# H2muller/CROPSR

Measured on AMD Instinct MI355X. Metric: gRNAs scored/sec, higher is better.
Workload: dtype f64

## Files before the change

cropsr_amd/csrc/crp_kernels.hip:

```cpp
#include <hip/hip_runtime.h>
#include <stdint.h>

#include <type_traits>

#include "crp_kernels.h"
#include "crp_score.h"
#include "crp_score_generic.h"

namespace crp {

static constexpr uint64_t ALL = ~0ull;

__device__ __forceinline__ uint32_t funnel(uint32_t hi, uint32_t lo, int s)
{
    return __builtin_amdgcn_alignbit(hi, lo, (uint32_t)s);
}
__device__ __forceinline__ uint64_t pair64(uint32_t hi, uint32_t lo) { return ((uint64_t)hi << 32) | lo; }

__device__ __forceinline__ uint64_t ahead(uint64_t cur, uint64_t next, int d)
{
    const uint32_t c0 = (uint32_t)cur, c1 = (uint32_t)(cur >> 32), n0 = (uint32_t)next, n1 = (uint32_t)(next >> 32);
    if (d < 32) return pair64(funnel(n0, c1, d), funnel(c1, c0, d));
    return pair64(funnel(n1, n0, d - 32), funnel(n0, c1, d - 32));
}
__device__ __forceinline__ uint64_t behind(uint64_t prev, uint64_t cur, int e)
{
    const uint32_t p0 = (uint32_t)prev, p1 = (uint32_t)(prev >> 32), c0 = (uint32_t)cur, c1 = (uint32_t)(cur >> 32);
    if (e == 32) return pair64(c0, p1);
    if (e < 32) return pair64(funnel(c1, c0, 32 - e), funnel(c0, p1, 32 - e));
    return pair64(funnel(c0, p1, 64 - e), funnel(p1, p0, 64 - e));
}

constexpr int DPP_WAVE_SHL1 = 0x130, DPP_WAVE_SHR1 = 0x138;
template <int CTRL>
__device__ __forceinline__ uint64_t wave_shift(uint64_t x, uint64_t edge)
{
    const uint32_t lo = (uint32_t)__builtin_amdgcn_update_dpp((int)(uint32_t)edge, (int)(uint32_t)x, CTRL, 0xf, 0xf, false);
    const uint32_t hi =
        (uint32_t)__builtin_amdgcn_update_dpp((int)(uint32_t)(edge >> 32), (int)(uint32_t)(x >> 32), CTRL, 0xf, 0xf, false);
    return pair64(hi, lo);
}

__device__ __forceinline__ uint64_t wave_inclusive_scan(uint64_t v)
{
    const int lane = threadIdx.x & 63;
#pragma unroll
    for (int d = 1; d < 64; d <<= 1) {
        const uint64_t o = __shfl_up(v, d, 64);
        if (lane >= d) v += o;
    }
    return v;
}

template <int CTRL, int ROW_MASK>
__device__ __forceinline__ uint32_t dpp_add(uint32_t v)
{
    return v + (uint32_t)__builtin_amdgcn_update_dpp(0, (int)v, CTRL, ROW_MASK, 0xf, true);
}

__device__ __forceinline__ uint32_t wave_inclusive_scan_u32(uint32_t v)
{
    v = dpp_add<0x111, 0xf>(v);
    v = dpp_add<0x112, 0xf>(v);
    v = dpp_add<0x114, 0xf>(v);
    v = dpp_add<0x118, 0xf>(v);
    v = dpp_add<0x142, 0xa>(v);
    v = dpp_add<0x143, 0xc>(v);
    return v;
}

__device__ __forceinline__ uint32_t wave_sum_u32(uint32_t v)
{
    return (uint32_t)__builtin_amdgcn_readlane((int)wave_inclusive_scan_u32(v), 63);
}

struct TileScan {
    uint32_t ex_plus, ex_minus, n_plus, n_minus;
};

template <int WAVES>
__device__ __forceinline__ TileScan block_exclusive_scan(uint32_t v16, uint32_t *wave_tot)
{
    const int lane = threadIdx.x & 63, wave = __builtin_amdgcn_readfirstlane((int)(threadIdx.x >> 6));
    const uint32_t inc16 = wave_inclusive_scan_u32(v16);
    if (lane == 63) wave_tot[wave] = inc16;
    __syncthreads();
    uint32_t base_p = 0, base_m = 0, tot_p = 0, tot_m = 0;
#pragma unroll
    for (int w = 0; w < WAVES; ++w) {
        const uint32_t t = (uint32_t)__builtin_amdgcn_readfirstlane((int)wave_tot[w]);
        if (w < wave) {
            base_p += t & 0xffffu;
            base_m += t >> 16;
        }
        tot_p += t & 0xffffu;
        tot_m += t >> 16;
    }
    const uint32_t ex16 = inc16 - v16;
    return TileScan{base_p + (ex16 & 0xffffu), base_m + (ex16 >> 16), tot_p, tot_m};
}

__device__ __forceinline__ void derive(uint64_t hi, uint64_t lo, uint64_t up, uint64_t ac, uint64_t &g,
                                       uint64_t &c, uint64_t &v)
{
    g = hi & lo & up & ac;
    c = hi & ~lo & up & ac;
    v = hi & lo & ~up & ~ac;
}

__device__ __forceinline__ void masks_of(uint64_t g_c, uint64_t g_n, uint64_t c_c, uint64_t c_n, uint64_t v_p,
                                         uint64_t v_c, uint64_t v_n, int l, uint64_t &mplus, uint64_t &mminus)
{
    mplus = ahead(g_c, g_n, 1) & ahead(g_c, g_n, 2) & ~behind(v_p, v_c, l + 5);
    uint64_t m = c_c & ahead(c_c, c_n, 1) & ~ahead(v_c, v_n, 2) & ~behind(v_p, v_c, 2);
    if (l > 8) m &= ~ahead(v_c, v_n, l - 8);
    mminus = m;
}

template <int WPT>
__device__ __forceinline__ void own_words_and_masks(const Planes &pl, uint64_t n_words_padded, uint64_t w0, int lane, int l,
                                                    uint64_t (&q)[4][WPT], uint64_t (&mp)[WPT], uint64_t (&mm)[WPT])
{
    static_assert(WPT == 1 || WPT == 2, "one or two words per owning lane");
    const uint64_t wa = w0 + (uint64_t)WPT * lane;
    if constexpr (WPT == 2) {
#pragma unroll
        for (int p = 0; p < 4; ++p) {
            const ulonglong2 v = *reinterpret_cast<const ulonglong2 *>(pl.plane[p] + wa);
            q[p][0] = v.x;
            q[p][WPT - 1] = v.y;
        }
    } else {
#pragma unroll
        for (int p = 0; p < 4; ++p) q[p][0] = pl.plane[p][wa];
    }
    uint64_t e[4] = {ALL, ALL, 0, 0};
    if (lane == 0 && w0 > 0) {
#pragma unroll
        for (int p = 0; p < 4; ++p) e[p] = pl.plane[p][w0 - 1];
    } else if (lane == 63 && w0 + 64 * WPT < n_words_padded) {
#pragma unroll
        for (int p = 0; p < 4; ++p) e[p] = pl.plane[p][w0 + 64 * WPT];
    }
    uint64_t ga, ca, va, gb, cb, vb, ge, ce, ve;
    derive(q[0][0], q[1][0], q[2][0], q[3][0], ga, ca, va);
    derive(q[0][WPT - 1], q[1][WPT - 1], q[2][WPT - 1], q[3][WPT - 1], gb, cb, vb);
    derive(e[0], e[1], e[2], e[3], ge, ce, ve);
    const uint64_t v_left = wave_shift<DPP_WAVE_SHR1>(vb, ve);
    const uint64_t g_right = wave_shift<DPP_WAVE_SHL1>(ga, ge), c_right = wave_shift<DPP_WAVE_SHL1>(ca, ce),
                   v_right = wave_shift<DPP_WAVE_SHL1>(va, ve);
    if constexpr (WPT == 2) {
        masks_of(ga, gb, ca, cb, v_left, va, vb, l, mp[0], mm[0]);
        masks_of(gb, g_right, cb, c_right, va, vb, v_right, l, mp[WPT - 1], mm[WPT - 1]);
    } else {
        masks_of(ga, g_right, ca, c_right, v_left, va, v_right, l, mp[0], mm[0]);
    }
}

template <class G, int LFIX>
__global__ __launch_bounds__(G::BLOCK) void count_kernel(Planes pl, uint64_t n_words_padded, int l_arg,
                                                         uint2 *__restrict__ tile_cnt)
{
    const int l = LFIX > 0 ? LFIX : l_arg;
    const uint32_t tile = blockIdx.x;
    __shared__ uint64_t wave_tot[G::BLOCK / 64];
    const int lane = threadIdx.x & 63, wave = threadIdx.x >> 6;
    uint64_t c = 0;
    const uint64_t w0 = (uint64_t)tile * G::WORDS + (uint64_t)wave * 64 * G::WPT;
    if (wave < G::OWNERS / 64 && w0 < n_words_padded) {
        uint64_t q[4][G::WPT], mp[G::WPT], mm[G::WPT];
        own_words_and_masks<G::WPT>(pl, n_words_padded, w0, lane, l, q, mp, mm);
#pragma unroll
        for (int k = 0; k < G::WPT; ++k) c += (uint64_t)__popcll(mp[k]) | ((uint64_t)__popcll(mm[k]) << 32);
    }
#pragma unroll
    for (int d = 32; d > 0; d >>= 1) c += __shfl_down(c, d, 64);
    if (lane == 0) wave_tot[wave] = c;
    __syncthreads();
    if (threadIdx.x == 0 && (uint64_t)tile * G::WORDS < n_words_padded) {
        uint64_t t = 0;
#pragma unroll
        for (int w = 0; w < G::BLOCK / 64; ++w) t += wave_tot[w];
        tile_cnt[tile] = make_uint2((uint32_t)t, (uint32_t)(t >> 32));
    }
}

__global__ __launch_bounds__(1024) void tile_scan_kernel(const uint2 *__restrict__ tile_cnt, uint32_t n_tiles,
                                                          uint2 *__restrict__ tile_off,
                                                          uint64_t *__restrict__ totals)
{
    const uint32_t chunk = blockIdx.x;
    constexpr int PER = 8, CHUNK = 1024 * PER;
    __shared__ uint64_t buf[CHUNK];
    __shared__ uint64_t wave_tot[16];
    const int lane = threadIdx.x & 63, wave = threadIdx.x >> 6;
    const uint32_t base = chunk * CHUNK;
    uint64_t carry = 0;
    {
        uint64_t acc = 0;
        const ulonglong2 *cnt2 = reinterpret_cast<const ulonglong2 *>(tile_cnt);
        for (uint32_t i = threadIdx.x; i < base / 2; i += 4096) {
            ulonglong2 c[4];
#pragma unroll
            for (int k = 0; k < 4; ++k) c[k] = cnt2[i + k * 1024];
#pragma unroll
            for (int k = 0; k < 4; ++k) {
                acc += c[k].x + c[k].y;
            }
        }
#pragma unroll
        for (int d = 32; d > 0; d >>= 1) acc += __shfl_xor(acc, d, 64);
        if (lane == 0) wave_tot[wave] = acc;
        __syncthreads();
#pragma unroll
        for (int w = 0; w < 16; ++w) carry += wave_tot[w];
        __syncthreads();
    }
    {
#pragma unroll
        for (int k = 0; k < PER; ++k) {
            const uint32_t i = base + k * 1024 + threadIdx.x;
            uint64_t v = 0;
            if (i < n_tiles) {
                const uint2 c = tile_cnt[i];
                v = (uint64_t)c.x | ((uint64_t)c.y << 32);
            }
            buf[k * 1024 + threadIdx.x] = v;
        }
        __syncthreads();
        uint64_t loc[PER], sum = 0;
#pragma unroll
        for (int k = 0; k < PER; ++k) {
            loc[k] = buf[threadIdx.x * PER + k];
            sum += loc[k];
        }
        const uint64_t inc = wave_inclusive_scan(sum);
        if (lane == 63) wave_tot[wave] = inc;
        __syncthreads();
        uint64_t pre = carry, tot = 0;
#pragma unroll
        for (int w = 0; w < 16; ++w) {
            const uint64_t t = wave_tot[w];
            if (w < wave) pre += t;
            tot += t;
        }
        uint64_t ex = pre + inc - sum;
#pragma unroll
        for (int k = 0; k < PER; ++k) {
            buf[threadIdx.x * PER + k] = ex;
            ex += loc[k];
        }
        carry += tot;
        __syncthreads();
#pragma unroll
        for (int k = 0; k < PER; ++k) {
            const uint32_t i = base + k * 1024 + threadIdx.x;
            const uint64_t v = buf[k * 1024 + threadIdx.x];
            if (i < n_tiles) tile_off[i] = make_uint2((uint32_t)v, (uint32_t)(v >> 32));
        }
    }
    if (threadIdx.x == 0 && base + CHUNK >= n_tiles) {
        totals[0] = carry & 0xffffffffull;
        totals[1] = carry >> 32;
    }
}

__device__ __forceinline__ uint32_t window31(const uint64_t *plane, uint32_t q)
{
    const uint32_t *p32 = reinterpret_cast<const uint32_t *>(plane);
    const uint32_t i = q >> 5;
    return __builtin_amdgcn_alignbit(p32[i + 1], p32[i], q & 31) & 0x7fffffffu;
}

__device__ __forceinline__ uint32_t window32(const uint64_t *plane, uint32_t q)
{
    const uint32_t *p32 = reinterpret_cast<const uint32_t *>(plane);
    const uint32_t i = q >> 5;
    return __builtin_amdgcn_alignbit(p32[i + 1], p32[i], q & 31);
}

__device__ __forceinline__ uint32_t reverse30(uint32_t x) { return __brev(x) >> 2; }

static constexpr uint64_t DESC_AGG = 1ull << 62, DESC_PREFIX = 2ull << 62, DESC_VALUE = (1ull << 62) - 1;

__device__ __forceinline__ uint64_t desc_pack(uint64_t packed32)
{
    return (packed32 & 0x7fffffffull) | ((packed32 >> 32) << 31);
}
__device__ __forceinline__ uint64_t desc_unpack(uint64_t v)
{
    return (v & 0x7fffffffull) | (((v >> 31) & 0x7fffffffull) << 32);
}

constexpr int CHAIN_HEADER_WORDS = 4;
constexpr int LB_DEPTH = 2;

__device__ __forceinline__ void lookback_publish(uint64_t *desc, uint32_t tile, uint64_t total)
{
    const uint64_t tag = tile == 0 ? DESC_PREFIX : DESC_AGG;
    __hip_atomic_store(&desc[tile], tag | desc_pack(total), __ATOMIC_RELAXED, __HIP_MEMORY_SCOPE_AGENT);
}

__device__ __forceinline__ void lookback_load(const uint64_t *desc, int64_t base, uint64_t (&v)[LB_DEPTH])
{
    const int lane = threadIdx.x & 63;
#pragma unroll
    for (int j = 0; j < LB_DEPTH; ++j) {
        const int64_t idx = base - lane - 64 * j;
        v[j] = DESC_PREFIX;
        if (idx >= 0) v[j] = __hip_atomic_load(&desc[idx], __ATOMIC_RELAXED, __HIP_MEMORY_SCOPE_AGENT);
    }
}

__device__ __forceinline__ uint64_t lookback_resolve(uint64_t *desc, uint32_t tile, uint64_t total, uint32_t *fail,
                                                     bool muted, uint32_t timeout_ticks)
{
    const int lane = threadIdx.x & 63;
    if (tile == 0) return 0;
    uint64_t v[LB_DEPTH];
    uint64_t excl = 0;
    int64_t base = (int64_t)tile - 1;
    lookback_load(desc, base, v);
    uint32_t spins = 0;
    uint64_t t_first_stall = 0;
    bool stalled_before = false;
    while (true) {
        uint64_t contrib = 0;
        bool found = false, stall = false;
        int64_t missing = 0;
#pragma unroll
        for (int j = 0; j < LB_DEPTH; ++j) {
            const uint64_t st = v[j] >> 62;
            const uint64_t not_ready = __ballot(st == 0);
            const uint64_t is_prefix = __ballot(st == 2);
            const int p = is_prefix ? __builtin_ctzll(is_prefix) : 64;
            const uint64_t need = p >= 64 ? ~0ull : ((1ull << p) - 1);
            if (!found && !stall) {
                if (not_ready & need) {
                    stall = true;
                    missing = base - 64 * j - __builtin_ctzll(not_ready & need);
                } else {
                    if (lane <= p) contrib += desc_unpack(v[j] & DESC_VALUE);
                    found = p < 64;
                }
            }
        }
        if (stall) {
            while ((__hip_atomic_load(&desc[missing], __ATOMIC_RELAXED, __HIP_MEMORY_SCOPE_AGENT) >> 62) == 0) {
                bool give_up = false;
                if ((spins++ & 15u) == 0) {
                    const uint64_t now = __builtin_amdgcn_s_memrealtime();
                    if (!stalled_before) {
                        t_first_stall = now;
                        stalled_before = true;
                    }
                    give_up = now - t_first_stall > timeout_ticks;
                    give_up |= __hip_atomic_load(fail, __ATOMIC_RELAXED, __HIP_MEMORY_SCOPE_AGENT) != 0;
                }
                if (give_up) {
                    if (lane == 0) {
                        atomicExch(fail, 1u);
                        uint64_t *const host = reinterpret_cast<uint64_t *>(reinterpret_cast<uint64_t *>(fail - 1)[3]);
                        if (host) host[0] = 1ull << 32;
                    }
                    return 0;
                }
                __builtin_amdgcn_s_sleep(8);
            }
        } else {
            excl += pair64(wave_sum_u32((uint32_t)(contrib >> 32)), wave_sum_u32((uint32_t)contrib));
            if (found) break;
            base -= 64 * LB_DEPTH;
        }
        lookback_load(desc, base, v);
    }
    if (lane == 0 && !muted)
        __hip_atomic_store(&desc[tile], DESC_PREFIX | desc_pack(excl + total), __ATOMIC_RELAXED, __HIP_MEMORY_SCOPE_AGENT);
    return excl;
}

struct ChainArgs {
    uint64_t *desc;
    uint32_t *fail;
    uint64_t *totals;
    uint64_t *s_excl;
    uint32_t *s_flag;
    uint32_t tile, n_tiles;
    uint64_t total;
    bool muted;
    uint32_t timeout_ticks;
};

__device__ __forceinline__ void chain_resolve(const ChainArgs &ch)
{
    const uint64_t e = lookback_resolve(ch.desc, ch.tile, ch.total, ch.fail, ch.muted, ch.timeout_ticks);
    if ((threadIdx.x & 63) == 0) {
        *ch.s_excl = e;
        if (ch.tile == ch.n_tiles - 1) {
            const uint64_t all = e + ch.total;
            ch.totals[0] = all & 0xffffffffull;
            ch.totals[1] = all >> 32;
            uint64_t *const host = reinterpret_cast<uint64_t *>(ch.totals[2]);
            if (host) {
                host[1] = all & 0xffffffffull;
                host[2] = all >> 32;
            }
        }
    }
    __hip_atomic_store(ch.s_flag, 1u, __ATOMIC_RELEASE, __HIP_MEMORY_SCOPE_WORKGROUP);
}

struct alignas(16) TabsImage {
    uint64_t exp_tab[256];
    double score_tab[CRP_SCORE_TAB_N];
};
static_assert(sizeof(TabsImage) % 16 == 0, "staged in 16-byte units");
__device__ const TabsImage CRP_TABS = {{
#include "exp_table.inc"
                                       },
                                       CRP_SCORE_TAB_DATA};

__device__ __forceinline__ __amdgpu_buffer_rsrc_t rows_rsrc(void *table, uint64_t cap, uint64_t first, uint32_t skip,
                                                            uint32_t elem)
{
    const uint64_t room = cap > first ? cap - first : 0;
    uint64_t bytes = room ? (room + skip) * elem : 0;
    if (bytes > 0xffffffffull) bytes = 0xffffffffull;
    char *base = reinterpret_cast<char *>(table) + ((int64_t)first - (int64_t)skip) * (int64_t)elem;
    return __builtin_amdgcn_make_buffer_rsrc(base, 0, (int)(uint32_t)bytes, 0x00020000);
}

struct TileStores {
    __amdgpu_buffer_rsrc_t pos[2], score[2], pre[2], seed[2];
};

constexpr int STORE_AUX = 2;
typedef uint32_t u32x2 __attribute__((__vector_size__(2 * sizeof(uint32_t))));
__device__ __forceinline__ u32x2 f64_words(double v)
{
    u32x2 w;
    w[0] = (uint32_t)__double2loint(v);
    w[1] = (uint32_t)__double2hiint(v);
    return w;
}

__device__ __forceinline__ uint64_t uniform64(uint64_t v)
{
    return ((uint64_t)(uint32_t)__builtin_amdgcn_readfirstlane((int)(v >> 32)) << 32) |
           (uint32_t)__builtin_amdgcn_readfirstlane((int)(uint32_t)v);
}

template <bool PRE, bool SEEDS>
__device__ __forceinline__ void tile_stores(TileStores &ts, const HitTables &out, uint64_t off_plus, uint64_t off_minus,
                                            uint32_t n_plus)
{
    ts.pos[0] = rows_rsrc(out.pos_plus, out.cap_plus, off_plus, 0, 4);
    ts.pos[1] = rows_rsrc(out.pos_minus, out.cap_minus, off_minus, n_plus, 4);
    ts.score[0] = rows_rsrc(out.score_plus, out.cap_plus, off_plus, 0, 8);
    ts.score[1] = rows_rsrc(out.score_minus, out.cap_minus, off_minus, n_plus, 8);
    if (PRE) {
        ts.pre[0] = rows_rsrc(out.pre_plus, out.cap_plus, off_plus, 0, 8);
        ts.pre[1] = rows_rsrc(out.pre_minus, out.cap_minus, off_minus, n_plus, 8);
    }
    if (SEEDS) {
        ts.seed[0] = rows_rsrc(out.seed_plus, out.cap_plus, off_plus, 0, 4);
        ts.seed[1] = rows_rsrc(out.seed_minus, out.cap_minus, off_minus, n_plus, 4);
    }
}

__device__ __forceinline__ void peel32(uint32_t m, uint32_t base, uint32_t &addr)
{
    uint32_t b, t;
    uint64_t saved;
    asm volatile(
        "s_mov_b64 %[saved], exec\n\t"
        "v_cmpx_ne_u32_e32 vcc, 0, %[m]\n\t"
        "s_cbranch_execz 2f\n"
        "1:\n\t"
        "v_ffbl_b32_e32 %[b], %[m]\n\t"
        "v_add_u32_e32 %[t], -1, %[m]\n\t"
        "v_or_b32_e32 %[b], %[b], %[base]\n\t"
        "v_and_b32_e32 %[m], %[t], %[m]\n\t"
        "ds_write_b16 %[addr], %[b]\n\t"
        "v_add_u32_e32 %[addr], 2, %[addr]\n\t"
        "v_cmpx_ne_u32_e32 vcc, 0, %[m]\n\t"
        "s_cbranch_execnz 1b\n"
        "2:\n\t"
        "s_mov_b64 exec, %[saved]"
        : [m] "+v"(m), [addr] "+v"(addr), [b] "=&v"(b), [t] "=&v"(t), [saved] "=&s"(saved)
        : [base] "v"(base)
        : "vcc", "memory");
}

template <class G, bool PAM, bool CHAINED, bool PRE, bool SEEDS>
__device__ __forceinline__ void emit_rounds(uint64_t (*sh)[G::WORDS + 2], uint16_t *list, uint64_t *exp_tab, double *score_tab,
                                            const uint64_t (&mp)[G::WPT], const uint64_t (&mm)[G::WPT], uint32_t ex_plus,
                                            uint32_t ex_minus,
                                            uint32_t n_plus, uint32_t n_minus, int l, uint32_t tile_pos,
                                            uint64_t off_plus, uint64_t off_minus, const HitTables &out,
                                            const ChainArgs &ch);

template <class G, bool CHAINED, int LFIX, bool PRE, bool SEEDS>
__global__ __launch_bounds__(G::BLOCK) __attribute__((amdgpu_waves_per_eu(6, 8))) void emit_kernel(
    Planes pl, uint64_t n_words_padded, int l_arg, const uint2 *__restrict__ tile_off, uint64_t *chain,
    uint64_t *__restrict__ chain_next, HitTables out, uint32_t mute_tile, uint32_t timeout_ticks)
{
    const int l = LFIX > 0 ? LFIX : l_arg;
    constexpr int TW = G::WORDS;
    __shared__ uint64_t sh[4][TW + 2];
    __shared__ __attribute__((aligned(16))) uint64_t tabs[256 + CRP_SCORE_TAB_N];
    uint64_t *const exp_tab = tabs;
    double *const score_tab = reinterpret_cast<double *>(tabs + 256);
    __shared__ uint32_t wave_tot[G::BLOCK / 64];
    __shared__ uint64_t s_excl;
    __shared__ uint32_t s_flag;
    __shared__ uint16_t list[G::LIST];
    static_assert(sizeof(sh) + sizeof(tabs) + sizeof(wave_tot) + sizeof(s_excl) + 8 + sizeof(list) <= G::LDS_LIMIT,
                  "workgroups per CU: see the geometry's LIST");

    const int tid = threadIdx.x;
    const uint32_t tile = blockIdx.x;
    if (CHAINED && tid == 0) s_flag = 0;
    const uint64_t t0 = (uint64_t)tile * TW;
    if (CHAINED) __builtin_amdgcn_s_setprio(3);
    uint64_t mp[G::WPT], mm[G::WPT];
#pragma unroll
    for (int k = 0; k < G::WPT; ++k) mp[k] = mm[k] = 0;
    if (G::OWNERS == G::BLOCK || tid < G::OWNERS) {
        const int lane = tid & 63;
        const uint64_t w0 = t0 + (uint64_t)(64 * G::WPT) * (uint64_t)(tid >> 6);
        uint64_t q[4][G::WPT];
        own_words_and_masks<G::WPT>(pl, n_words_padded, w0, lane, l, q, mp, mm);
#pragma unroll
        for (int p = 0; p < 4; ++p)
#pragma unroll
            for (int k = 0; k < G::WPT; ++k) sh[p][1 + G::WPT * tid + k] = q[p][k];
        if (tid < 8) {
            const int p = tid >> 1;
            const uint64_t voidw = (p < 2) ? ALL : 0ull;
            if (tid & 1) sh[p][TW + 1] = t0 + TW < n_words_padded ? pl.plane[p][t0 + TW] : voidw;
            else sh[p][0] = t0 > 0 ? pl.plane[p][t0 - 1] : voidw;
        }
    }
    uint32_t c16 = 0;
#pragma unroll
    for (int k = 0; k < G::WPT; ++k) c16 += (uint32_t)__popcll(mp[k]) | ((uint32_t)__popcll(mm[k]) << 16);
    const TileScan sc = block_exclusive_scan<G::BLOCK / 64>(c16, wave_tot);
    const uint32_t n_plus = sc.n_plus, n_minus = sc.n_minus;
    const uint32_t n_all = n_plus + n_minus;
    const uint64_t total = pair64(n_minus, n_plus);
    uint64_t off_plus = 0, off_minus = 0;
    ChainArgs ch{};
    if (CHAINED) {
        ch = ChainArgs{chain + CHAIN_HEADER_WORDS, reinterpret_cast<uint32_t *>(chain) + 1, chain + 1, &s_excl, &s_flag,
                       tile, gridDim.x, total, tile == mute_tile, timeout_ticks};
        if (tid == 0) {
            if (tile != mute_tile) lookback_publish(ch.desc, tile, total);
            chain_next[CHAIN_HEADER_WORDS + tile] = 0;
            if (tile == 0) chain_next[0] = chain_next[1] = chain_next[2] = 0;
        }
        __builtin_amdgcn_s_setprio(0);
        if (n_all == 0) {
            if (tile == ch.n_tiles - 1 && tid < 64) chain_resolve(ch);
            return;
        }
    } else {
        const uint2 off = tile_off[tile];
        off_plus = off.x;
        off_minus = off.y;
        if (n_all == 0) return;
    }
    constexpr uint32_t TAB_UNITS = (LFIX == 20 ? sizeof(TabsImage) : sizeof(CRP_TABS.exp_tab)) / 16;
    for (uint32_t k = tid; k < TAB_UNITS; k += G::BLOCK)
        reinterpret_cast<uint4 *>(tabs)[k] = reinterpret_cast<const uint4 *>(&CRP_TABS)[k];
    emit_rounds<G, LFIX == 20, CHAINED, PRE, SEEDS>(sh, list, exp_tab, score_tab, mp, mm, sc.ex_plus, sc.ex_minus, n_plus, n_minus, l,
                                                 (uint32_t)(t0 * 64),
                                                 off_plus, off_minus, out, ch);
}

template <class G, bool PAM, bool CHAINED, bool PRE, bool SEEDS>
__device__ __forceinline__ void emit_rounds(uint64_t (*sh)[G::WORDS + 2], uint16_t *list, uint64_t *exp_tab, double *score_tab,
                                            const uint64_t (&mp)[G::WPT], const uint64_t (&mm)[G::WPT], uint32_t ex_plus,
                                            uint32_t ex_minus,
                                            uint32_t n_plus, uint32_t n_minus, int l, uint32_t tile_pos,
                                            uint64_t off_plus, uint64_t off_minus, const HitTables &out,
                                            const ChainArgs &ch)
{
    constexpr uint32_t CAP = G::LIST;
    const int tid = threadIdx.x;
    const uint32_t n_all = n_plus + n_minus;
    TileStores ts;
    bool resolved = !CHAINED;
    if (!CHAINED) tile_stores<PRE, SEEDS>(ts, out, uniform64(off_plus), uniform64(off_minus), n_plus);
    const bool by_strand = n_all > CAP && n_plus <= CAP && n_minus <= CAP;
    const uint32_t list_lds = (uint32_t)(uintptr_t)list;
    uint32_t hi_rank = 0;
    for (uint32_t lo_rank = 0; lo_rank < n_all; lo_rank = hi_rank) {
        hi_rank = by_strand ? (lo_rank == 0 ? n_plus : n_all) : min(lo_rank + CAP, n_all);
        if (lo_rank) __syncthreads();
        const uint32_t rp0 = ex_plus - lo_rank;
        const uint32_t rm0 = ex_minus + (n_plus - lo_rank);
        if (n_all <= CAP || by_strand) {
            const bool with_plus = !by_strand || lo_rank == 0, with_minus = !by_strand || lo_rank != 0;
            uint32_t ap = list_lds + 2 * rp0, am = list_lds + 2 * rm0;
            if (G::OWNERS == G::BLOCK || tid < G::OWNERS) {
#pragma unroll
                for (int k = 0; k < G::WPT; ++k) {
                    const uint32_t wbase = (uint32_t)(tid * G::WPT + k) * 64u;
                    if (with_plus) {
                        peel32((uint32_t)mp[k], wbase, ap);
                        peel32((uint32_t)(mp[k] >> 32), wbase + 32, ap);
                    }
                    if (with_minus) {
                        peel32((uint32_t)mm[k], wbase, am);
                        peel32((uint32_t)(mm[k] >> 32), wbase + 32, am);
                    }
                }
            }
        } else {
            uint32_t rp = rp0, rm = rm0;
#pragma unroll
            for (int k = 0; k < G::WPT; ++k) {
                const uint32_t wbase = (uint32_t)(tid * G::WPT + k) * 64u;
                for (uint64_t m = mp[k]; m; m &= m - 1, ++rp)
                    if (rp < CAP) list[rp] = (uint16_t)(wbase + __builtin_ctzll(m));
                for (uint64_t m = mm[k]; m; m &= m - 1, ++rm)
                    if (rm < CAP) list[rm] = (uint16_t)(wbase + __builtin_ctzll(m));
            }
        }
        __syncthreads();
        const uint32_t n_round = hi_rank - lo_rank;
        struct Hit {
            uint32_t e, r, seed;
            double pre, score;
        };
        struct Fetched {
            uint32_t e, r, h, w, u, a;
        };
        auto fetch = [&](uint32_t k) -> Fetched {
            Fetched f{list[k], lo_rank + k, 0, 0, 0, 0};
            const uint32_t q = 64u + f.e - (f.r >= n_plus ? 2u : PAM ? 27u : (uint32_t)(l + 5));
            if (PAM) {
                f.h = window32(sh[0], q);
                f.w = window32(sh[1], q);
                f.u = window32(sh[2], q);
                f.a = window32(sh[3], q);
            } else if (l >= 20) {
                f.h = window31(sh[0], q);
                f.w = window31(sh[1], q);
                f.u = window31(sh[2], q);
                f.a = window31(sh[3], q);
            }
            return f;
        };
        auto score = [&](const Fetched &f) -> Hit {
            Hit hit{f.e, f.r, SEED_RAW_NONE, -1.0, -1.0};
            const bool minus = hit.r >= n_plus;
            if (PAM) {
                const uint32_t u = f.u;
                uint32_t h = f.h, w = f.w, valid = f.a | u;
                if (!minus) {
                    h = __brev(h);
                    w = __brev(w ^ u);
                    valid = __brev(valid);
                }
                const bool complete = (h & w & ~valid & 0x3fffffffu) == 0;
                if (SEEDS) {
                    if (((valid >> 5) & 0xfffu) == 0xfffu) hit.seed = (((h >> 5) & 0xfffu) << 12) | ((w >> 5) & 0xfffu);
                }
                if (complete) {
                    const uint32_t mG = h & w, mC = h & ~w;
                    const uint32_t mT = ~h & w, mA = ~h & ~w & valid;
                    crp_score_masks<PAM>(mA, mT, mC, mG, exp_tab, score_tab, hit.pre, hit.score);
                }
            } else if (l >= 20) {
                uint32_t h = f.h, w = f.w, u = f.u, a = f.a;
                const uint32_t vd = h & w & ~u & ~a;
                const bool complete = (vd & 0x3fffffffu) == 0 && (l == 20 || (vd >> 30));
                h &= 0x3fffffffu;
                w &= 0x3fffffffu;
                u &= 0x3fffffffu;
                a &= 0x3fffffffu;
                uint32_t valid = a | u;
                if (!minus) {
                    h = reverse30(h);
                    w = reverse30(w ^ u);
                    valid = reverse30(valid);
                }
                static_assert(!SEEDS || PAM, "seed words are emitted by the l = 20 variant only");
                if (complete) {
                    const uint32_t mG = h & w & valid, mC = h & ~w & valid;
                    const uint32_t mT = ~h & w & valid, mA = ~h & ~w & valid;
                    crp_score_masks<PAM>(mA, mT, mC, mG, exp_tab, score_tab, hit.pre, hit.score);
                }
            }
            return hit;
        };
        auto store = [&](const Hit &hit) {
            const uint32_t pos = tile_pos + hit.e;
            const int o4 = (int)(hit.r * 4u), o8 = (int)(hit.r * 8u);
            const bool minus = hit.r >= n_plus;
#pragma unroll
            for (int st = 0; st < 2; ++st) {
                if (minus == (st == 1)) {
                    __builtin_amdgcn_raw_buffer_store_b32(pos, ts.pos[st], o4, 0, STORE_AUX);
                    __builtin_amdgcn_raw_buffer_store_b64(f64_words(hit.score), ts.score[st], o8, 0, STORE_AUX);
                    if (PRE) __builtin_amdgcn_raw_buffer_store_b64(f64_words(hit.pre), ts.pre[st], o8, 0, STORE_AUX);
                    if (SEEDS) __builtin_amdgcn_raw_buffer_store_b32(hit.seed, ts.seed[st], o4, 0, STORE_AUX);
                    if (st == 0) asm volatile("; '+' rows stored" ::: "memory");
                    else asm volatile("; '-' rows stored" ::: "memory");
                }
            }
        };
        auto run_rows = [&](uint32_t k, auto before_first_store) {
            const bool any = k < n_round;
            Hit first{};
            if (any) first = score(fetch(k));
            before_first_store(any);
            if (any) {
                store(first);
                for (k += G::BLOCK; k < n_round; k += G::BLOCK) store(score(fetch(k)));
            }
        };
        if (!CHAINED) {
            run_rows(tid, [](bool) {});
        } else {
            const uint32_t k0 = (uint32_t)(tid & 63) | ((((uint32_t)tid >> 6) + (G::BLOCK / 64 - 1)) % (G::BLOCK / 64)) << 6;
            if (lo_rank == 0 && tid < 64) chain_resolve(ch);
            run_rows(k0, [&](bool any) {
                if (!resolved && __ballot(any)) {
                    while (__builtin_amdgcn_readfirstlane((int)__hip_atomic_load(ch.s_flag, __ATOMIC_ACQUIRE, __HIP_MEMORY_SCOPE_WORKGROUP)) == 0)
                        __builtin_amdgcn_s_sleep(1);
                    const uint64_t e = uniform64(*ch.s_excl);
                    tile_stores<PRE, SEEDS>(ts, out, e & 0xffffffffull, e >> 32, n_plus);
                    resolved = true;
                }
            });
        }
    }
}

__global__ __launch_bounds__(BLOCK) void score30_kernel(const uint8_t *__restrict__ rows, uint64_t n,
                                                         double *__restrict__ pre_out,
                                                         double *__restrict__ score_out)
{
    __shared__ uint64_t exp_tab[256];
    exp_tab[threadIdx.x] = CRP_EXP_TAB[threadIdx.x];
    __syncthreads();
    for (uint64_t i = (uint64_t)blockIdx.x * BLOCK + threadIdx.x; i < n; i += (uint64_t)gridDim.x * BLOCK) {
        const uint8_t *r = rows + 30 * i;
        uint32_t mA = 0, mT = 0, mC = 0, mG = 0;
#pragma unroll
        for (int p = 0; p < 30; ++p) {
            const uint32_t ch = r[p];
            mA |= (uint32_t)(ch == 'A') << p;
            mT |= (uint32_t)(ch == 'T') << p;
            mC |= (uint32_t)(ch == 'C') << p;
            mG |= (uint32_t)(ch == 'G') << p;
        }
        double pre, score;
        crp_score_masks<false>(mA, mT, mC, mG, exp_tab, nullptr, pre, score);
        if (pre_out) pre_out[i] = pre;
        score_out[i] = score;
    }
}

__global__ __launch_bounds__(64) void score30_order_kernel(const uint8_t *__restrict__ rows, uint64_t n, int order,
                                                            double *__restrict__ pre_out,
                                                            double *__restrict__ score_out)
{
    __shared__ uint64_t exp_tab[256];
    for (int k = threadIdx.x; k < 256; k += 64) exp_tab[k] = CRP_EXP_TAB[k];
    __syncthreads();
    for (uint64_t i = (uint64_t)blockIdx.x * 64 + threadIdx.x; i < n; i += (uint64_t)gridDim.x * 64) {
        int8_t code[30];
        for (int p = 0; p < 30; ++p) {
            const uint32_t ch = rows[30 * i + p];
            code[p] = ch == 'A' ? 0 : ch == 'T' ? 1 : ch == 'C' ? 2 : ch == 'G' ? 3 : -1;
        }
        double s1, s2;
        if (order == CRP_ORDER_TAIL2) {
            s1 = crp_sum_tail2<false>(code);
            s2 = crp_sum_tail2<true>(code);
        } else {
            s1 = crp_sum_dot1<false>(code);
            s2 = crp_sum_dot1<true>(code);
        }
        const double pre = (((s1 + s2) + CRP_INTERSECT) + CRP_LOW_GC) * -1.0;
        if (pre_out) pre_out[i] = pre;
        score_out[i] = 1.0 / (1.0 + crp_exp(pre, exp_tab));
    }
}

__host__ __device__ inline uint8_t classify_char(uint32_t ch)
{
    switch (ch) {
        case 'A': case 'U': return 0xC;
        case 'T': return 0xE;
        case 'C': return 0xD;
        case 'G': return 0xF;
        case 'a': return 0x8;
        case 't': return 0xA;
        case 'c': return 0x9;
        case 'g': return 0xB;
        case 'Z': return 0x5;
        default:  return 0x0;
    }
}

__global__ __launch_bounds__(BLOCK) void pack_kernel(const uint8_t *__restrict__ text, uint64_t len,
                                                      uint64_t n_words, uint64_t *__restrict__ hi,
                                                      uint64_t *__restrict__ lo, uint64_t *__restrict__ up,
                                                      uint64_t *__restrict__ ac)
{
    __shared__ uint8_t lut[256];
    __shared__ __attribute__((aligned(16))) uint8_t buf[BLOCK / 64][4096];
    const int tid = threadIdx.x, lane = tid & 63, wave = tid >> 6;
    lut[tid] = classify_char(tid);
    const uint64_t n_groups = (n_words + 63) / 64;
    const uint64_t n_block_iters = (n_groups + BLOCK / 64 - 1) / (BLOCK / 64);
    for (uint64_t bi = blockIdx.x; bi < n_block_iters; bi += gridDim.x) {
        const uint64_t group = bi * (BLOCK / 64) + wave;
        const uint64_t base = group * 4096;
        __syncthreads();
        if (group < n_groups) {
#pragma unroll
            for (int it = 0; it < 4; ++it) {
                const uint64_t off = base + (uint64_t)it * 1024 + (uint64_t)lane * 16;
                uint4 v = make_uint4(0, 0, 0, 0);
                if (off + 16 <= len) {
                    v = *reinterpret_cast<const uint4 *>(text + off);
                } else if (off < len) {
                    uint8_t tmp[16];
                    for (int b = 0; b < 16; ++b) tmp[b] = off + b < len ? text[off + b] : 0;
                    v = *reinterpret_cast<const uint4 *>(tmp);
                }
                *reinterpret_cast<uint4 *>(&buf[wave][it * 1024 + lane * 16]) = v;
            }
        }
        __syncthreads();
        if (group < n_groups) {
            uint64_t w_hi = 0, w_lo = 0, w_up = 0, w_ac = 0;
            for (int t = 0; t < 64; ++t) {
                const uint64_t idx = base + (uint64_t)t * 64 + lane;
                const uint32_t nib = idx < len ? lut[buf[wave][t * 64 + lane]] : 0x3u;
                const uint64_t b0 = __ballot(nib & 1), b1 = __ballot(nib & 2);
                const uint64_t b2 = __ballot(nib & 4), b3 = __ballot(nib & 8);
                if (lane == t) { w_hi = b0; w_lo = b1; w_up = b2; w_ac = b3; }
            }
            const uint64_t w = group * 64 + lane;
            if (w < n_words) { hi[w] = w_hi; lo[w] = w_lo; up[w] = w_up; ac[w] = w_ac; }
        }
    }
}

__global__ __launch_bounds__(BLOCK) void pack_groups_kernel(const uint8_t *__restrict__ text, const PackGroup *__restrict__ groups,
                                                             uint32_t n_groups, uint64_t *__restrict__ hi, uint64_t *__restrict__ lo,
                                                             uint64_t *__restrict__ up, uint64_t *__restrict__ ac)
{
    __shared__ uint8_t lut[256];
    __shared__ __attribute__((aligned(16))) uint8_t buf[BLOCK / 64][4096];
    const int tid = threadIdx.x, lane = tid & 63, wave = tid >> 6;
    lut[tid] = classify_char(tid);
    const uint32_t n_iters = (n_groups + BLOCK / 64 - 1) / (BLOCK / 64);
    for (uint32_t it = blockIdx.x; it < n_iters; it += gridDim.x) {
        const uint32_t g = it * (BLOCK / 64) + wave;
        __syncthreads();
        PackGroup pg{0, 0, 0, 0, 0};
        if (g < n_groups) {
            pg = groups[g];
#pragma unroll
            for (int k = 0; k < 4; ++k)
                *reinterpret_cast<uint4 *>(&buf[wave][k * 1024 + lane * 16]) =
                    *reinterpret_cast<const uint4 *>(text + pg.src + (uint32_t)k * 1024 + (uint32_t)lane * 16);
        }
        __syncthreads();
        if (g < n_groups) {
            uint64_t w_hi = 0, w_lo = 0, w_up = 0, w_ac = 0;
            for (uint32_t t = 0; t < pg.n_words; ++t) {
                const uint32_t idx = t * 64 + lane;
                const uint32_t nib = idx < pg.n_chars ? lut[buf[wave][idx]] : 0x3u;
                const uint64_t b0 = __ballot(nib & 1), b1 = __ballot(nib & 2);
                const uint64_t b2 = __ballot(nib & 4), b3 = __ballot(nib & 8);
                if ((uint32_t)lane == t) { w_hi = b0; w_lo = b1; w_up = b2; w_ac = b3; }
            }
            if ((uint32_t)lane < pg.n_words) {
                const uint64_t w = pg.dst_word + lane;
                hi[w] = w_hi;
                lo[w] = w_lo;
                up[w] = w_up;
                ac[w] = w_ac;
            }
        }
    }
}

template <class G>
static hipError_t launch_count_geo(hipStream_t s, const Planes &pl, uint64_t n_words_padded, int l, uint2 *tile_cnt, uint32_t n_tiles)
{
    if (l == 20)
        hipLaunchKernelGGL((count_kernel<G, 20>), dim3(n_tiles), dim3(G::BLOCK), 0, s, pl, n_words_padded, l, tile_cnt);
    else
        hipLaunchKernelGGL((count_kernel<G, 0>), dim3(n_tiles), dim3(G::BLOCK), 0, s, pl, n_words_padded, l, tile_cnt);
    return hipGetLastError();
}

#define CRP_BY_GEOMETRY(geo, CALL)                 \
    switch (geo) {                                 \
        case GEO_LARGE: return CALL(GeoLarge);     \
        case GEO_SMALL: return CALL(GeoSmall);     \
        default: return hipErrorInvalidValue;      \
    }

hipError_t launch_count(hipStream_t s, int geo, const Planes &pl, uint64_t n_words_padded, int l, uint2 *tile_cnt,
                        uint32_t n_tiles)
{
    if (n_tiles == 0) return hipSuccess;
#define CRP_CALL(G) launch_count_geo<G>(s, pl, n_words_padded, l, tile_cnt, n_tiles)
    CRP_BY_GEOMETRY(geo, CRP_CALL)
#undef CRP_CALL
}

hipError_t launch_tile_scan(hipStream_t s, const uint2 *tile_cnt, uint32_t n_tiles, uint2 *tile_off, uint64_t *totals)
{
    if (n_tiles == 0) return hipSuccess;
    const uint32_t n_chunks = (n_tiles + SCAN_CHUNK_TILES - 1) / SCAN_CHUNK_TILES;
    hipLaunchKernelGGL(tile_scan_kernel, dim3(n_chunks), dim3(1024), 0, s, tile_cnt, n_tiles, tile_off, totals);
    return hipGetLastError();
}

template <class G, bool CHAINED>
static hipError_t launch_emit_variant(hipStream_t s, const Planes &pl, uint64_t n_words_padded, int l, const uint2 *tile_off,
                                      uint64_t *chain, uint64_t *chain_next, const HitTables &out, uint32_t mute_tile,
                                      uint32_t timeout_ticks)
{
    const uint32_t n_tiles = (uint32_t)(n_words_padded / G::WORDS);
    if (n_tiles == 0) return hipSuccess;
    const bool pre = out.pre_plus != nullptr, seeds = out.seed_plus != nullptr;
    if (seeds && l != 20) return hipErrorInvalidValue;
#define CRP_LAUNCH(LFIX, PRE, SEEDS)                                                                                       \
    hipLaunchKernelGGL((emit_kernel<G, CHAINED, LFIX, PRE, SEEDS>), dim3(n_tiles), dim3(G::BLOCK), 0, s, pl, n_words_padded, l, \
                       tile_off, chain, chain_next, out, mute_tile, timeout_ticks)
    if (l == 20) {
        if (seeds) {
            if (pre) CRP_LAUNCH(20, true, true);
            else CRP_LAUNCH(20, false, true);
        } else {
            if (pre) CRP_LAUNCH(20, true, false);
            else CRP_LAUNCH(20, false, false);
        }
    } else {
        if (pre) CRP_LAUNCH(0, true, false);
        else CRP_LAUNCH(0, false, false);
    }
#undef CRP_LAUNCH
    return hipGetLastError();
}

hipError_t launch_emit(hipStream_t s, int geo, const Planes &pl, uint64_t n_words_padded, int l, const uint2 *tile_off,
                       const HitTables &out)
{
#define CRP_CALL(G) launch_emit_variant<G, false>(s, pl, n_words_padded, l, tile_off, nullptr, nullptr, out, 0xffffffffu, 0u)
    CRP_BY_GEOMETRY(geo, CRP_CALL)
#undef CRP_CALL
}

size_t chain_bytes(uint32_t n_tiles) { return (CHAIN_HEADER_WORDS + (size_t)n_tiles) * sizeof(uint64_t); }

hipError_t launch_emit_chained(hipStream_t s, int geo, const Planes &pl, uint64_t n_words_padded, int l, uint64_t *chain,
                               uint64_t *chain_next, const HitTables &out, uint32_t mute_tile, uint32_t timeout_ticks)
{
#define CRP_CALL(G) launch_emit_variant<G, true>(s, pl, n_words_padded, l, nullptr, chain, chain_next, out, mute_tile, timeout_ticks)
    CRP_BY_GEOMETRY(geo, CRP_CALL)
#undef CRP_CALL
}

int tile_words(int geo) { return geo == GEO_SMALL ? GeoSmall::WORDS : GeoLarge::WORDS; }

hipError_t launch_score30(hipStream_t s, const uint8_t *rows, uint64_t n, int order, double *pre, double *score)
{
    if (n == 0) return hipSuccess;
    if (order != CRP_ORDER_BODY4) {
        const uint64_t b = (n + 63) / 64;
        hipLaunchKernelGGL(score30_order_kernel, dim3((uint32_t)(b < 1024 ? b : 1024)), dim3(64), 0, s, rows, n,
                           order, pre, score);
        return hipGetLastError();
    }
    const uint64_t blocks = (n + BLOCK - 1) / BLOCK;
    const uint32_t grid = (uint32_t)(blocks < 8192 ? blocks : 8192);
    hipLaunchKernelGGL(score30_kernel, dim3(grid), dim3(BLOCK), 0, s, rows, n, pre, score);
    return hipGetLastError();
}

hipError_t launch_pack_groups(hipStream_t s, const uint8_t *text, const PackGroup *groups, uint32_t n_groups, uint64_t *hi,
                              uint64_t *lo, uint64_t *up, uint64_t *ac)
{
    if (n_groups == 0) return hipSuccess;
    const uint32_t iters = (n_groups + BLOCK / 64 - 1) / (BLOCK / 64);
    hipLaunchKernelGGL(pack_groups_kernel, dim3(iters < 4096 ? iters : 4096), dim3(BLOCK), 0, s, text, groups, n_groups, hi, lo, up, ac);
    return hipGetLastError();
}

hipError_t launch_pack(hipStream_t s, const uint8_t *text, uint64_t len, uint64_t n_words, uint64_t *hi,
                       uint64_t *lo, uint64_t *up, uint64_t *ac)
{
    if (n_words == 0) return hipSuccess;
    const uint64_t iters = ((n_words + 63) / 64 + BLOCK / 64 - 1) / (BLOCK / 64);
    const uint32_t grid = (uint32_t)(iters < 4096 ? iters : 4096);
    hipLaunchKernelGGL(pack_kernel, dim3(grid), dim3(BLOCK), 0, s, text, len, n_words, hi, lo, up, ac);
    return hipGetLastError();
}

__global__ __launch_bounds__(BLOCK) void count_scored_kernel(const double *__restrict__ score, uint64_t n,
                                                              unsigned long long *__restrict__ out)
{
    uint64_t c = 0;
    for (uint64_t i = (uint64_t)blockIdx.x * BLOCK + threadIdx.x; i < n; i += (uint64_t)gridDim.x * BLOCK)
        c += score[i] != -1.0;
#pragma unroll
    for (int d = 32; d > 0; d >>= 1) c += __shfl_down(c, d, 64);
    if ((threadIdx.x & 63) == 0 && c) atomicAdd(out, (unsigned long long)c);
}

hipError_t launch_count_scored(hipStream_t s, const double *score, uint64_t n, uint64_t *out)
{
    if (n == 0) return hipSuccess;
    const uint64_t blocks = (n + BLOCK - 1) / BLOCK;
    hipLaunchKernelGGL(count_scored_kernel, dim3((uint32_t)(blocks < 2048 ? blocks : 2048)), dim3(BLOCK), 0, s, score, n,
                       reinterpret_cast<unsigned long long *>(out));
    return hipGetLastError();
}

__global__ __launch_bounds__(BLOCK) void count_plain_kernel(const uint64_t *__restrict__ up, const uint64_t *__restrict__ ac,
                                                             uint64_t n_words, unsigned long long *__restrict__ out)
{
    uint64_t c = 0;
    for (uint64_t w = (uint64_t)blockIdx.x * BLOCK + threadIdx.x; w < n_words; w += (uint64_t)gridDim.x * BLOCK)
        c += (uint64_t)__popcll(up[w] & ac[w]);
#pragma unroll
    for (int d = 32; d > 0; d >>= 1) c += __shfl_down(c, d, 64);
    if ((threadIdx.x & 63) == 0 && c) atomicAdd(out, (unsigned long long)c);
}

hipError_t launch_count_plain(hipStream_t s, const uint64_t *up, const uint64_t *ac, uint64_t n_words, uint64_t *out)
{
    if (n_words == 0) return hipSuccess;
    const uint64_t blocks = (n_words + BLOCK - 1) / BLOCK;
    hipLaunchKernelGGL(count_plain_kernel, dim3((uint32_t)(blocks < 2048 ? blocks : 2048)), dim3(BLOCK), 0, s, up, ac, n_words,
                       reinterpret_cast<unsigned long long *>(out));
    return hipGetLastError();
}

uint8_t host_classify_char(uint32_t ch) { return classify_char(ch); }

}
```

Baseline: 126.7 billion.

## Pad plus-strand hits to wave boundary so each wave scores a single strand

Lays out the LDS hit list so minus-strand entries start at a 64-aligned offset after the plus entries. Each wave then processes rows of only one strand, with strand as a compile-time type, which removes per-lane strand selection and divergent store branches. Rounds are split per strand, and the chained-offset resolution is moved to a per-wave first trip. This adds padding slots and some wasted lanes, and it changes the row-offset bookkeeping for the minus-strand buffers.

```diff
diff --git a/cropsr_amd/csrc/crp_kernels.hip b/cropsr_amd/csrc/crp_kernels.hip
--- a/cropsr_amd/csrc/crp_kernels.hip
+++ b/cropsr_amd/csrc/crp_kernels.hip
@@ -452,19 +452,19 @@
 
 template <bool PRE, bool SEEDS>
 __device__ __forceinline__ void tile_stores(TileStores &ts, const HitTables &out, uint64_t off_plus, uint64_t off_minus,
-                                            uint32_t n_plus)
+                                            uint32_t minus_row0)
 {
     ts.pos[0] = rows_rsrc(out.pos_plus, out.cap_plus, off_plus, 0, 4);
-    ts.pos[1] = rows_rsrc(out.pos_minus, out.cap_minus, off_minus, n_plus, 4);
+    ts.pos[1] = rows_rsrc(out.pos_minus, out.cap_minus, off_minus, minus_row0, 4);
     ts.score[0] = rows_rsrc(out.score_plus, out.cap_plus, off_plus, 0, 8);
-    ts.score[1] = rows_rsrc(out.score_minus, out.cap_minus, off_minus, n_plus, 8);
+    ts.score[1] = rows_rsrc(out.score_minus, out.cap_minus, off_minus, minus_row0, 8);
     if (PRE) {
         ts.pre[0] = rows_rsrc(out.pre_plus, out.cap_plus, off_plus, 0, 8);
-        ts.pre[1] = rows_rsrc(out.pre_minus, out.cap_minus, off_minus, n_plus, 8);
+        ts.pre[1] = rows_rsrc(out.pre_minus, out.cap_minus, off_minus, minus_row0, 8);
     }
     if (SEEDS) {
         ts.seed[0] = rows_rsrc(out.seed_plus, out.cap_plus, off_plus, 0, 4);
-        ts.seed[1] = rows_rsrc(out.seed_minus, out.cap_minus, off_minus, n_plus, 4);
+        ts.seed[1] = rows_rsrc(out.seed_minus, out.cap_minus, off_minus, minus_row0, 4);
     }
 }
 
@@ -586,80 +586,68 @@
                                             uint64_t off_plus, uint64_t off_minus, const HitTables &out,
                                             const ChainArgs &ch)
 {
-    constexpr uint32_t CAP = G::LIST;
+    constexpr uint32_t CAP = G::LIST, NW = G::BLOCK / 64;
     const int tid = threadIdx.x;
-    const uint32_t n_all = n_plus + n_minus;
+    const uint32_t lane = (uint32_t)tid & 63u, wave = (uint32_t)__builtin_amdgcn_readfirstlane(tid >> 6);
+    const uint32_t n_plus_pad = (n_plus + 63u) & ~63u;
     TileStores ts;
     bool resolved = !CHAINED;
-    if (!CHAINED) tile_stores<PRE, SEEDS>(ts, out, uniform64(off_plus), uniform64(off_minus), n_plus);
-    const bool by_strand = n_all > CAP && n_plus <= CAP && n_minus <= CAP;
+    if (!CHAINED) tile_stores<PRE, SEEDS>(ts, out, uniform64(off_plus), uniform64(off_minus), n_plus_pad);
+    const uint32_t n_all = n_plus + n_minus;
+    const bool single = n_plus_pad + n_minus <= CAP;
     const uint32_t list_lds = (uint32_t)(uintptr_t)list;
     uint32_t hi_rank = 0;
     for (uint32_t lo_rank = 0; lo_rank < n_all; lo_rank = hi_rank) {
-        hi_rank = by_strand ? (lo_rank == 0 ? n_plus : n_all) : min(lo_rank + CAP, n_all);
-        if (lo_rank) __syncthreads();
-        const uint32_t rp0 = ex_plus - lo_rank;
-        const uint32_t rm0 = ex_minus + (n_plus - lo_rank);
-        if (n_all <= CAP || by_strand) {
-            const bool with_plus = !by_strand || lo_rank == 0, with_minus = !by_strand || lo_rank != 0;
-            uint32_t ap = list_lds + 2 * rp0, am = list_lds + 2 * rm0;
-            if (G::OWNERS == G::BLOCK || tid < G::OWNERS) {
+        const bool first_round = lo_rank == 0;
+        const bool plus_round = lo_rank < n_plus;
+        hi_rank = single ? n_all : min(lo_rank + CAP, plus_round ? n_plus : n_all);
+        const uint32_t p_lo = min(lo_rank, n_plus), m_lo = lo_rank - p_lo;
+        const uint32_t np_r = min(hi_rank, n_plus) - p_lo, nm_r = hi_rank - lo_rank - np_r;
+        const uint32_t m_at = (np_r + 63u) & ~63u;
+        if (!first_round) __syncthreads();
+        const uint32_t rp0 = ex_plus - p_lo;
+        const uint32_t rm0 = ex_minus - m_lo + m_at;
+        if (G::OWNERS == G::BLOCK || tid < G::OWNERS) {
+            if (n_plus <= CAP && n_minus <= CAP) {
+                uint32_t ap = list_lds + 2 * rp0, am = list_lds + 2 * rm0;
 #pragma unroll
                 for (int k = 0; k < G::WPT; ++k) {
                     const uint32_t wbase = (uint32_t)(tid * G::WPT + k) * 64u;
-                    if (with_plus) {
+                    if (np_r) {
                         peel32((uint32_t)mp[k], wbase, ap);
                         peel32((uint32_t)(mp[k] >> 32), wbase + 32, ap);
                     }
-                    if (with_minus) {
+                    if (nm_r) {
                         peel32((uint32_t)mm[k], wbase, am);
                         peel32((uint32_t)(mm[k] >> 32), wbase + 32, am);
                     }
                 }
+            } else {
+                uint32_t rp = rp0, rm = rm0 - m_at;
+#pragma unroll
+                for (int k = 0; k < G::WPT; ++k) {
+                    const uint32_t wbase = (uint32_t)(tid * G::WPT + k) * 64u;
+                    for (uint64_t m = mp[k]; m; m &= m - 1, ++rp)
+                        if (rp < np_r) list[rp] = (uint16_t)(wbase + __builtin_ctzll(m));
+                    for (uint64_t m = mm[k]; m; m &= m - 1, ++rm)
+                        if (rm < nm_r) list[m_at + rm] = (uint16_t)(wbase + __builtin_ctzll(m));
+                }
             }
-        } else {
-            uint32_t rp = rp0, rm = rm0;
-#pragma unroll
-            for (int k = 0; k < G::WPT; ++k) {
-                const uint32_t wbase = (uint32_t)(tid * G::WPT + k) * 64u;
-                for (uint64_t m = mp[k]; m; m &= m - 1, ++rp)
-                    if (rp < CAP) list[rp] = (uint16_t)(wbase + __builtin_ctzll(m));
-                for (uint64_t m = mm[k]; m; m &= m - 1, ++rm)
-                    if (rm < CAP) list[rm] = (uint16_t)(wbase + __builtin_ctzll(m));
-            }
         }
         __syncthreads();
-        const uint32_t n_round = hi_rank - lo_rank;
+        const uint32_t row0_plus = p_lo, row0_minus = n_plus_pad + m_lo - m_at;
         struct Hit {
-            uint32_t e, r, seed;
+            uint32_t e, seed;
             double pre, score;
         };
-        struct Fetched {
-            uint32_t e, r, h, w, u, a;
-        };
-        auto fetch = [&](uint32_t k) -> Fetched {
-            Fetched f{list[k], lo_rank + k, 0, 0, 0, 0};
-            const uint32_t q = 64u + f.e - (f.r >= n_plus ? 2u : PAM ? 27u : (uint32_t)(l + 5));
+        auto score = [&](auto strand, uint32_t k) -> Hit {
+            constexpr bool MINUS = decltype(strand)::value;
+            Hit hit{list[k], SEED_RAW_NONE, -1.0, -1.0};
+            const uint32_t q = 64u + hit.e - (MINUS ? 2u : PAM ? 27u : (uint32_t)(l + 5));
             if (PAM) {
-                f.h = window32(sh[0], q);
-                f.w = window32(sh[1], q);
-                f.u = window32(sh[2], q);
-                f.a = window32(sh[3], q);
-            } else if (l >= 20) {
-                f.h = window31(sh[0], q);
-                f.w = window31(sh[1], q);
-                f.u = window31(sh[2], q);
-                f.a = window31(sh[3], q);
-            }
-            return f;
-        };
-        auto score = [&](const Fetched &f) -> Hit {
-            Hit hit{f.e, f.r, SEED_RAW_NONE, -1.0, -1.0};
-            const bool minus = hit.r >= n_plus;
-            if (PAM) {
-                const uint32_t u = f.u;
-                uint32_t h = f.h, w = f.w, valid = f.a | u;
-                if (!minus) {
+                const uint32_t u = window32(sh[2], q);
+                uint32_t h = window32(sh[0], q), w = window32(sh[1], q), valid = window32(sh[3], q) | u;
+                if (!MINUS) {
                     h = __brev(h);
                     w = __brev(w ^ u);
                     valid = __brev(valid);
@@ -674,7 +662,7 @@
                     crp_score_masks<PAM>(mA, mT, mC, mG, exp_tab, score_tab, hit.pre, hit.score);
                 }
             } else if (l >= 20) {
-                uint32_t h = f.h, w = f.w, u = f.u, a = f.a;
+                uint32_t h = window31(sh[0], q), w = window31(sh[1], q), u = window31(sh[2], q), a = window31(sh[3], q);
                 const uint32_t vd = h & w & ~u & ~a;
                 const bool complete = (vd & 0x3fffffffu) == 0 && (l == 20 || (vd >> 30));
                 h &= 0x3fffffffu;
@@ -682,7 +670,7 @@
                 u &= 0x3fffffffu;
                 a &= 0x3fffffffu;
                 uint32_t valid = a | u;
-                if (!minus) {
+                if (!MINUS) {
                     h = reverse30(h);
                     w = reverse30(w ^ u);
                     valid = reverse30(valid);
@@ -696,47 +684,42 @@
             }
             return hit;
         };
-        auto store = [&](const Hit &hit) {
-            const uint32_t pos = tile_pos + hit.e;
-            const int o4 = (int)(hit.r * 4u), o8 = (int)(hit.r * 8u);
-            const bool minus = hit.r >= n_plus;
-#pragma unroll
-            for (int st = 0; st < 2; ++st) {
-                if (minus == (st == 1)) {
-                    __builtin_amdgcn_raw_buffer_store_b32(pos, ts.pos[st], o4, 0, STORE_AUX);
-                    __builtin_amdgcn_raw_buffer_store_b64(f64_words(hit.score), ts.score[st], o8, 0, STORE_AUX);
-                    if (PRE) __builtin_amdgcn_raw_buffer_store_b64(f64_words(hit.pre), ts.pre[st], o8, 0, STORE_AUX);
-                    if (SEEDS) __builtin_amdgcn_raw_buffer_store_b32(hit.seed, ts.seed[st], o4, 0, STORE_AUX);
-                    if (st == 0) asm volatile("; '+' rows stored" ::: "memory");
-                    else asm volatile("; '-' rows stored" ::: "memory");
-                }
-            }
+        auto store = [&](auto strand, const Hit &hit, uint32_t k) {
+            constexpr int st = decltype(strand)::value ? 1 : 0;
+            const uint32_t pos = tile_pos + hit.e, r = k + (st ? row0_minus : row0_plus);
+            const int o4 = (int)(r * 4u), o8 = (int)(r * 8u);
+            __builtin_amdgcn_raw_buffer_store_b32(pos, ts.pos[st], o4, 0, STORE_AUX);
+            __builtin_amdgcn_raw_buffer_store_b64(f64_words(hit.score), ts.score[st], o8, 0, STORE_AUX);
+            if (PRE) __builtin_amdgcn_raw_buffer_store_b64(f64_words(hit.pre), ts.pre[st], o8, 0, STORE_AUX);
+            if (SEEDS) __builtin_amdgcn_raw_buffer_store_b32(hit.seed, ts.seed[st], o4, 0, STORE_AUX);
+            if (st == 0) asm volatile("; '+' rows stored" ::: "memory");
+            else asm volatile("; '-' rows stored" ::: "memory");
         };
-        auto run_rows = [&](uint32_t k, auto before_first_store) {
-            const bool any = k < n_round;
-            Hit first{};
-            if (any) first = score(fetch(k));
-            before_first_store(any);
-            if (any) {
-                store(first);
-                for (k += G::BLOCK; k < n_round; k += G::BLOCK) store(score(fetch(k)));
-            }
+        uint32_t cb = (CHAINED ? (wave + (NW - 1)) % NW : wave) << 6;
+        if (CHAINED && first_round && tid < 64) chain_resolve(ch);
+        auto trip = [&](auto strand, uint32_t end, auto before_store) {
+            const uint32_t k = cb + lane;
+            const bool act = k < end;
+            Hit hit;
+            if (act) hit = score(strand, k);
+            before_store();
+            if (act) store(strand, hit, k);
+            cb += G::BLOCK;
         };
-        if (!CHAINED) {
-            run_rows(tid, [](bool) {});
-        } else {
-            const uint32_t k0 = (uint32_t)(tid & 63) | ((((uint32_t)tid >> 6) + (G::BLOCK / 64 - 1)) % (G::BLOCK / 64)) << 6;
-            if (lo_rank == 0 && tid < 64) chain_resolve(ch);
-            run_rows(k0, [&](bool any) {
-                if (!resolved && __ballot(any)) {
-                    while (__builtin_amdgcn_readfirstlane((int)__hip_atomic_load(ch.s_flag, __ATOMIC_ACQUIRE, __HIP_MEMORY_SCOPE_WORKGROUP)) == 0)
-                        __builtin_amdgcn_s_sleep(1);
-                    const uint64_t e = uniform64(*ch.s_excl);
-                    tile_stores<PRE, SEEDS>(ts, out, e & 0xffffffffull, e >> 32, n_plus);
-                    resolved = true;
-                }
-            });
-        }
+        if (CHAINED) {
+            auto pick_up = [&]() {
+                if (resolved) return;
+                while (__builtin_amdgcn_readfirstlane((int)__hip_atomic_load(ch.s_flag, __ATOMIC_ACQUIRE, __HIP_MEMORY_SCOPE_WORKGROUP)) == 0)
+                    __builtin_amdgcn_s_sleep(1);
+                const uint64_t e = uniform64(*ch.s_excl);
+                tile_stores<PRE, SEEDS>(ts, out, e & 0xffffffffull, e >> 32, n_plus_pad);
+                resolved = true;
+            };
+            if (cb < np_r) trip(std::false_type{}, np_r, pick_up);
+            else if (cb < m_at + nm_r) trip(std::true_type{}, m_at + nm_r, pick_up);
+        }
+        while (cb < np_r) trip(std::false_type{}, np_r, []() {});
+        while (cb < m_at + nm_r) trip(std::true_type{}, m_at + nm_r, []() {});
     }
 }
 
```

New measurement: 125.6 billion. About the same (-0.8%).
